# erikszasz/GaussianSplattingRegistration

Hardware: AMD Instinct MI355X
Metric: Gaussians/sec through HEM level + ICP iters/sec, 2x5M-splat pair (higher is better)
Workload: dtype f32 (HEM) / f64 (ICP)

## Files before the change

gaussiansplattingregistration_amd/csrc/hem_select.h:

```cpp
#pragma once
#include "hem_device.h"

namespace gsr {

struct ParentRec;
struct SelectArgs {
    const float4* A;
    const float4* geo;
    const float* Rs;
    const unsigned* plist;
    const unsigned* porder;
    int xcd;
    const int* nheavy;
    int own_lo, own_hi;
    const int* cellStart;
    const float4* Ac;
    const int* cellStartC;
    const int* cellStartI;
    const double* logtab;
    const int* irank;
    const unsigned* ipos;
    int n_irr;
    int ell;
    const GridParams* gp;
    int P;
    float colorThr2;
    float kldThr, tau2;
    const ParentRec* prec;
    unsigned* pcnt;
    unsigned* pcap;
    const int64_t* poff;
    unsigned* pair_child;
    float* pair_wl;
    const uint2* hitem;
    const int* hfirst;
    unsigned* part_cnt;
    int* hq;
    int heavy_blocks;
    const unsigned* part_p;
    unsigned long long cap_pairs;
    int* abort_p;
    int np;
    int2* rowlist;
};

enum { SEL_COUNT = 0, SEL_FILL = 1, SEL_SPARSE = 2 };
#define SEL_PART 8192
#define SEL_HEAVY_BLOCKS 2048
#define SEL_QCAP 256
#define SEL_U 3
#define SEL_MCAP 1024
#define SEL_ROWS 16
#define SEL_PAD (64 * SEL_U)

struct EllClip {
    float on;
    float k11, k12, k22, kr, im00, m01, m02, T;
};
struct ParentRec {
    f3 pm, pcol;
    s6 pinv;
    float det_p, inv_det_p, pweight, R, R2;
    float white;
    float u00, u01, u02, u11, u12, u22;
    float T1;
    EllClip ec;
    int js;
    int active;
    int selfq;
    float ey, ez;
    int rows;
};
static_assert(sizeof(ParentRec) == 160, "ParentRec is fetched as 40 dwords");

__device__ __forceinline__ float fast_sqrt(float x) { return __builtin_amdgcn_sqrtf(x); }

__device__ __forceinline__ int mbcnt64(unsigned long long mask, int base) {
    return (int)__builtin_amdgcn_mbcnt_hi((unsigned)(mask >> 32), __builtin_amdgcn_mbcnt_lo((unsigned)mask, (unsigned)base));
}
__device__ __forceinline__ unsigned long long uniform64(unsigned long long v) {
    return ((unsigned long long)(unsigned)__builtin_amdgcn_readfirstlane((int)(v >> 32)) << 32) |
           (unsigned)__builtin_amdgcn_readfirstlane((int)v);
}
__device__ __forceinline__ int wave_incl_scan(int v) {
    v += __builtin_amdgcn_update_dpp(0, v, 0x111, 0xf, 0xf, false);
    v += __builtin_amdgcn_update_dpp(0, v, 0x112, 0xf, 0xf, false);
    v += __builtin_amdgcn_update_dpp(0, v, 0x114, 0xf, 0xf, false);
    v += __builtin_amdgcn_update_dpp(0, v, 0x118, 0xf, 0xf, false);
    v += __builtin_amdgcn_update_dpp(0, v, 0x142, 0xa, 0xf, false);
    v += __builtin_amdgcn_update_dpp(0, v, 0x143, 0xc, 0xf, false);
    return v;
}

#ifdef GSR_SELECT_PROFILE
extern __device__ unsigned long long g_sel_prof[1024 * 16];
#define SEL_PROF_T(var) const unsigned long long var = __builtin_amdgcn_s_memtime()
#define SEL_PROF_ADD(slot, t0, lane) do { if ((lane) == 0) atomicAdd(&g_sel_prof[(blockIdx.x & 1023u) * 16 + (slot)], __builtin_amdgcn_s_memtime() - (t0)); } while (0)
#define SEL_PROF_CNT(slot, v, lane) do { if ((lane) == 0) atomicAdd(&g_sel_prof[(blockIdx.x & 1023u) * 16 + (slot)], (unsigned long long)(v)); } while (0)
#else
#define SEL_PROF_T(var)
#define SEL_PROF_ADD(slot, t0, lane)
#define SEL_PROF_CNT(slot, v, lane)
#endif

__device__ __forceinline__ bool kl_gate_rejects(float s2, float det_c, float det_p, float inv_det_p, float thr, const double* logtab,
                                                float* lf_out = nullptr, bool* exact_out = nullptr) {
    const float qf = det_c * inv_det_p;
    const float lf = __builtin_amdgcn_logf(qf) * 0.6931471805599453f;
    const float kf = 0.5f * (s2 - lf);
    const float margin = 1e-6f * (1.0f + fabsf(lf) + fabsf(s2));
    bool reject = kf > thr;
    const bool need_exact = !(qf >= 4.0f * FLT_MIN && qf <= 0.25f * FLT_MAX) || !(fabsf(s2) <= FLT_MAX) || !(fabsf(kf - thr) > margin);
    if (need_exact) {
        const float k = 0.5f * (s2 - glibc_logf_tab(det_c / det_p, logtab));
        reject = k > thr;
    }
    if (lf_out) *lf_out = lf;
    if (exact_out) *exact_out = need_exact;
    return reject;
}


template <bool IRR>
__device__ __forceinline__ void select_row_span(const SelectArgs& a, const GridParams& g, const f3& pm, const EllClip& ec, bool clip,
                                                float Ra2, int x0, int x1, int ry, int rz, int& s, int& len) {
    const bool edge = ry == 0 || ry == g.gy - 1 || rz == 0 || rz == g.gz - 1;
    const float ylo = ry == 0 ? -FLT_MAX : g.oy + ry * g.c - g.slack, yhi = ry == g.gy - 1 ? FLT_MAX : g.oy + (ry + 1) * g.c + g.slack;
    const float zlo = rz == 0 ? -FLT_MAX : g.oz + rz * g.c - g.slack, zhi = rz == g.gz - 1 ? FLT_MAX : g.oz + (rz + 1) * g.c + g.slack;
    const float dy = fmaxf(0.0f, fmaxf(ylo - pm.y, pm.y - yhi));
    const float dz = fmaxf(0.0f, fmaxf(zlo - pm.z, pm.z - zhi));
    const float rem = Ra2 - dy * dy - dz * dz;
    if (rem >= 0.0f) {
        const float hx = fast_sqrt(rem) * 1.00001f + g.slack;
        float lo = -hx, hi = hx;
        if (clip && !edge) {
            const float cy = 0.5f * (ylo + yhi) - pm.y, cz = 0.5f * (zlo + zhi) - pm.z;
            const float hy = 0.5f * (yhi - ylo), hz = 0.5f * (zhi - zlo);
            const float sc = fast_sqrt(fmaxf(0.0f, ec.k11 * cy * cy + 2.0f * ec.k12 * cy * cz + ec.k22 * cz * cz));
            const float smin = fmaxf(0.0f, sc * 0.999f - ec.kr * fast_sqrt(hy * hy + hz * hz));
            const float rem2 = ec.T - smin * smin;
            if (rem2 < 0.0f) {
                lo = 1.0f; hi = -1.0f;
            } else {
                const float w = fast_sqrt(rem2 * ec.im00) * 1.001f;
                const float t1 = ec.m01 * cy, t2 = ec.m02 * cz;
                const float xc = -(t1 + t2) * ec.im00;
                const float dl = (fabsf(ec.m01) * hy + fabsf(ec.m02) * hz) * ec.im00 * 1.001f;
                const float pad = g.slack + 1e-5f * fabsf(xc) + 1e-6f * (fabsf(t1) + fabsf(t2)) * ec.im00;
                lo = fmaxf(lo, xc - dl - w - pad);
                hi = fminf(hi, xc + dl + w + pad);
            }
        }
        if (lo <= hi) {
            int xa = cell_of(pm.x + lo, g.ox, g.inv_c, g.gx), xb = cell_of(pm.x + hi, g.ox, g.inv_c, g.gx);
            xa = xa < x0 ? x0 : xa;
            xb = xb > x1 ? x1 : xb;
            const int rowbase = (rz * g.gy + ry) * g.gx;
            int e;
            if (IRR) { s = a.cellStartI[rowbase + xa]; e = a.cellStartI[rowbase + xb + 1]; }
            else { s = a.cellStartC[rowbase + xa]; e = a.cellStartC[rowbase + xb + 1]; }
            len = e - s;
        }
    }
}

__device__ __forceinline__ void make_filter(const s6& Mf, float det_p, float kldThr, int ell, bool parent_regular, ParentRec& pr) {
    EllClip ec;
    ec.on = 0.0f; ec.k11 = ec.k12 = ec.k22 = ec.kr = ec.im00 = ec.m01 = ec.m02 = 0.0f; ec.T = __builtin_inff();
    pr.white = 0.0f;
    pr.u00 = pr.u01 = pr.u02 = pr.u11 = pr.u12 = pr.u22 = 0.0f;
    pr.T1 = __builtin_inff();
    pr.ey = pr.ez = __builtin_inff();
    const double thr2 = 2.0 * (double)kldThr;
    if (parent_regular && thr2 >= 0.0 && thr2 < 1e30) {
        const double m00 = Mf.e00, m01 = Mf.e01, m02 = Mf.e02, m11 = Mf.e11, m12 = Mf.e12, m22 = Mf.e22;
        double detM;
        const bool finite = fabs(m00) < 1e30 && fabs(m01) < 1e30 && fabs(m02) < 1e30 && fabs(m11) < 1e30 && fabs(m12) < 1e30 && fabs(m22) < 1e30;
        if (finite && spd_det64(m00, m01, m02, m11, m12, m22, detM)) {
            const double trM = m00 + m11 + m22;
            const double e2 = (m00 * m11 - m01 * m01) + (m00 * m22 - m02 * m02) + (m11 * m22 - m12 * m12);
            const double K = trM * e2 / detM * 1.000001;
            const double u = 5.9604644775390625e-8;
            const double theta = 6.1 * u * K + 2.0 * u;
            const double G = -(log(detM) + log((double)det_p)) + 2e-6;
            if (theta <= 0.25 && fabs(G) <= 1.0) {
                const double smin = (thr2 * (1.0 + 2.0 * u) + G + (double)GSR_DET_TOL + 3.2 * theta / (1.0 - theta) + 4e-5) / (1.0 - theta);
                const double T1 = smin * (1.0 + theta) * (1.0 + theta) * (1.0 + 1e-5);
                if (T1 > 0.0 && T1 < 1e30) {
                    const double u00 = sqrt(m00), u01 = m01 / u00, u02 = m02 / u00;
                    const double t11 = m11 - u01 * u01, u11 = sqrt(t11), u12 = (m12 - u01 * u02) / u11;
                    const double t22 = m22 - u02 * u02 - u12 * u12, u22 = sqrt(t22);
                    if (t11 > 0.0 && t22 > 0.0) {
                        pr.u00 = (float)u00; pr.u01 = (float)u01; pr.u02 = (float)u02; pr.u11 = (float)u11; pr.u12 = (float)u12; pr.u22 = (float)u22;
                        pr.T1 = (float)(T1 * (1.0 + 2.0 * u));
                        pr.white = 1.0f;
                        if (ell) {
                            const double Tc = T1 * (1.0 + theta) * (1.0 + theta) * (1.0 + 1e-4);
                            const double fk = 1.0 - 4.0 * theta - 2e-3;
                            const double im00 = 1.0 / m00;
                            const double k11 = (m11 - m01 * m01 * im00) * fk, k12 = (m12 - m01 * m02 * im00) * fk, k22 = (m22 - m02 * m02 * im00) * fk;
                            ec.k11 = (float)k11; ec.k12 = (float)k12; ec.k22 = (float)k22;
                            ec.kr = (float)(sqrt((k11 + k22) / fk) * 1.001);
                            ec.im00 = (float)(im00 * (1.0 + 4.0 * u));
                            ec.m01 = (float)m01; ec.m02 = (float)m02;
                            ec.T = (float)(Tc * (1.0 + 2.0 * u));
                            const bool ok = fk > 0.5 && k11 > 0.0 && k22 > 0.0 && k11 * k22 > k12 * k12 && ec.kr < FLT_MAX && ec.im00 < FLT_MAX && ec.T < FLT_MAX;
                            ec.on = ok ? 1.0f : 0.0f;
                            pr.ey = (float)(sqrt(fmax(0.0, Tc * (m00 * m22 - m02 * m02) / detM)) * 1.001);
                            pr.ez = (float)(sqrt(fmax(0.0, Tc * (m00 * m11 - m01 * m01) / detM)) * 1.001);
                        }
                    }
                }
            }
        }
    }
    pr.ec = ec;
}

__device__ __forceinline__ float white_smd(const float (&vc)[11], float cx, float cy, float cz) {
    const float dx = cx - vc[0], dy = cy - vc[1], dz = cz - vc[2];
    const float y2 = vc[8] * dz;
    const float y1 = __builtin_fmaf(vc[6], dy, vc[7] * dz);
    const float y0 = __builtin_fmaf(vc[3], dx, __builtin_fmaf(vc[4], dy, vc[5] * dz));
    return __builtin_fmaf(y0, y0, __builtin_fmaf(y1, y1, y2 * y2));
}

#define SEL_NP 4
#define SEL_TAG_SHIFT 30
#define SEL_TAG_MASK 0x3fffffffu

void launch_parent_prep(hipStream_t st, int P, const unsigned* plist, const float4* geo, const float* Rs, float kldThr, int ell, ParentRec* prec);
void launch_spans(hipStream_t st, const SelectArgs& sa);
int32_t launch_select(int mode, const SelectArgs& sa, hipStream_t st, hipStream_t aux, hipEvent_t ev_fork, hipEvent_t ev_join);
constexpr int SEL_WPB = 2;
void select_set_attributes();
int32_t select_profile(unsigned long long* out16, int32_t reset);

}
```

gaussiansplattingregistration_amd/csrc/hem_select.hip:

```cpp
#include "hem_select.h"

namespace gsr {

#ifdef GSR_SELECT_PROFILE
__device__ unsigned long long g_sel_prof[1024 * 16];
#endif
struct __attribute__((aligned(16))) ParLds {
    float4 r0;
    float4 r1;
    float4 r2;
    float4 r3;
    float R2;
    int js;
    int64_t base;
};
static_assert(sizeof(ParLds) == 80, "ParLds is read as four float4 and two 8-byte words");

#define SEL_Q3CAP 128
struct Q3 {
    unsigned *j, *rel;
    float *d2, *cd, *op, *det;
    int h, n;
};

__device__ __forceinline__ void select_stage3(const SelectArgs& a, const ParLds* par, int lane, int cnt, Q3& q3) {
    if (lane < cnt) {
        const int k = (q3.h + lane) & (SEL_Q3CAP - 1);
        const unsigned e = q3.j[k];
        const ParLds* pl = par + (e >> SEL_TAG_SHIFT);
        const float distanceDiff = sqrtf(q3.d2[k]);
        const float cdiff = sqrtf(q3.cd[k]);
        const float distWeight = expf(-distanceDiff * distanceDiff / a.tau2);
        const float colorInfluence = expf(-cdiff * cdiff / a.tau2);
        const float L = distWeight * q3.op[k] * colorInfluence * sqrtf(q3.det[k]);
        const int64_t dst = pl->base + (int64_t)q3.rel[k];
        a.pair_child[dst] = e & SEL_TAG_MASK;
        a.pair_wl[dst] = pl->r3.z * ref_clamp(L, FLT_MIN, 1e8f);
    }
    q3.h = (q3.h + cnt) & (SEL_Q3CAP - 1);
    q3.n -= cnt;
}

template <int MODE>
__device__ __forceinline__ void select_stage2(const SelectArgs& a, const ParLds* par, int lane, int cnt, const unsigned* q, int qh,
                                              unsigned& count_v, Q3& q3) {
    SEL_PROF_T(tp2);
    SEL_PROF_CNT(8, 1, lane); SEL_PROF_CNT(9, cnt, lane);
    bool acc = false;
    unsigned e = 0u;
    int k = 0;
    float d2 = 0.0f, cdiff = 0.0f, op = 0.0f, det_c = 0.0f;
    if (lane < cnt) {
        e = q[(qh + lane) & (SEL_QCAP - 1)];
        const int j = (int)(e & SEL_TAG_MASK);
        k = (int)(e >> SEL_TAG_SHIFT);
        const ParLds* pl = par + k;
        const float4 p0 = pl->r0, p1 = pl->r1;
        const float R2 = pl->R2;
        const float4* row = a.geo + 4 * (int64_t)j;
        float4 ca = row[0], cb = row[1], cc = row[2], cd = row[3];
        asm volatile("" : "+v"(ca.x), "+v"(ca.y), "+v"(ca.z), "+v"(ca.w), "+v"(cb.x), "+v"(cb.y), "+v"(cb.z), "+v"(cb.w),
                          "+v"(cc.x), "+v"(cc.y), "+v"(cc.z), "+v"(cc.w), "+v"(cd.x), "+v"(cd.y), "+v"(cd.z), "+v"(cd.w));
        const f3 cm = {ca.x, ca.y, ca.z};
        const f3 ccol = {cc.z, cc.w, cd.x};
        const f3 pm = {p0.x, p0.y, p0.z}, pcol = {p0.w, p1.x, p1.y};
        const f3 d = sub3(cm, pm);
        d2 = dot3(d, d);
        const f3 dc = sub3(ccol, pcol);
        cdiff = dot3(dc, dc);
        if (d2 < R2 && !(cdiff > a.colorThr2)) {
            const float4 p2 = pl->r2, p3 = pl->r3;
            const s6 ccov = {cb.x, cb.y, cb.z, cb.w, cc.x, cc.y};
            const s6 pinv = {p1.z, p1.w, p2.x, p2.y, p2.z, p2.w};
            det_c = cd.w;
            op = cd.y;
            const float smd = dot3(d, mul6(pinv, d));
            const float tr = trace_prod6(pinv, ccov);
            const float s2 = smd + tr - 3.0f;
            if (!kl_gate_rejects(s2, det_c, p3.x, p3.y, a.kldThr, a.logtab)) {
                const bool child_is_parent = (__float_as_uint(ca.w) & 1u) != 0u;
                acc = !(child_is_parent && j != pl->js);
            }
        }
    }
    const unsigned long long m = __ballot(acc);
    const int na = __popcll(m);
    SEL_PROF_CNT(15, na, lane);
    if (na == 0) { SEL_PROF_ADD(2, tp2, lane); return; }
    const int k_lo = __builtin_amdgcn_readfirstlane(k);
    const int k_hi = __builtin_amdgcn_readlane(k, __builtin_amdgcn_readfirstlane(cnt - 1));
    unsigned rel = 0u;
#pragma unroll
    for (int kk = 0; kk < SEL_NP; ++kk) {
        if (kk < k_lo || kk > k_hi) continue;
        const unsigned long long mk = __ballot(acc && k == kk);
        const unsigned ck = (unsigned)__builtin_amdgcn_readlane((int)count_v, kk);
        if (acc && k == kk) rel = ck + (unsigned)mbcnt64(mk, 0);
        if (lane == kk) count_v += (unsigned)__popcll(mk);
    }
    if (MODE == SEL_COUNT) { SEL_PROF_ADD(2, tp2, lane); return; }
    if (acc) {
        const int t = mbcnt64(m, q3.h + q3.n) & (SEL_Q3CAP - 1);
        q3.j[t] = e; q3.rel[t] = rel; q3.d2[t] = d2; q3.cd[t] = cdiff; q3.op[t] = op; q3.det[t] = det_c;
    }
    q3.n += na;
    __builtin_amdgcn_wave_barrier();
    if (q3.n >= 64) select_stage3(a, par, lane, 64, q3);
    __builtin_amdgcn_wave_barrier();
    SEL_PROF_ADD(2, tp2, lane);
}

__global__ __launch_bounds__(256) void k_parent_prep(int P, const unsigned* __restrict__ plist, const float4* __restrict__ geo,
                                                     const float* __restrict__ Rs, float kldThr, int ell, ParentRec* __restrict__ prec) {
    __shared__ ParentRec s_pr[4][64];
    const int lane = threadIdx.x & 63, wv = threadIdx.x >> 6;
    for (int base = blockIdx.x * blockDim.x + (threadIdx.x & ~63); base < P; base += gridDim.x * blockDim.x) {
        const int p = base + lane;
        if (p < P) {
        ParentRec pr;
        pr.js = (int)plist[p];
        const float4* prow = geo + 4 * (int64_t)pr.js;
        const float4 pa = prow[0], pb = prow[1], pc = prow[2], pd = prow[3];
        pr.pm = {pa.x, pa.y, pa.z};
        pr.det_p = pd.w;
        pr.inv_det_p = 1.0f / pd.w;
        const s6 pcov = {pb.x, pb.y, pb.z, pb.w, pc.x, pc.y};
        pr.pcol = {pc.z, pc.w, pd.x};
        pr.pweight = pd.z;
        pr.pinv = inverse6(pcov, pr.det_p);
        pr.R = Rs[pr.js];
        pr.R2 = pr.R * pr.R;
        make_filter(pr.pinv, pr.det_p, kldThr, ell, (__float_as_uint(pa.w) & 2u) != 0u, pr);
        const bool pm_finite = fabsf(pr.pm.x) <= FLT_MAX && fabsf(pr.pm.y) <= FLT_MAX && fabsf(pr.pm.z) <= FLT_MAX;
        pr.active = (pr.R2 > 0.0f && pm_finite) ? 1 : 0;
        pr.selfq = (pr.active && (__float_as_uint(pa.w) & 2u)) ? 1 : 0;
        pr.rows = 0;
        s_pr[wv][lane] = pr;
        }
        __builtin_amdgcn_wave_barrier();
        const int nrec = P - base < 64 ? P - base : 64;
        const float4* src = reinterpret_cast<const float4*>(s_pr[wv]);
        float4* dst = reinterpret_cast<float4*>(prec + base);
        for (int t = lane; t < nrec * (int)(sizeof(ParentRec) / 16); t += 64) dst[t] = src[t];
        __builtin_amdgcn_wave_barrier();
    }
}

template <int MODE, bool IRR>
__device__ __forceinline__ void select_scan(const SelectArgs& a, const GridParams& g, const ParentRec& pr, const ParLds* par, unsigned ktag,
                                            const float (&vc)[11], int lane, unsigned long long* bits, unsigned* q, int& qh, int& qn, unsigned& count_v,
                                            Q3& q3, unsigned& cum, unsigned lo, unsigned hi, const int2* rl, int lcnt) {
    const f3 pm = pr.pm;
    const EllClip& ec = pr.ec;
    const bool listed = rl != nullptr;
    bool clip = false;
    int x0 = 0, x1 = 0, y0 = 0, z0 = 0, ny = 1, nrows = lcnt;
    float Ra2 = 0.0f;
    if (!listed) {
        int vz;
        asm volatile("v_mov_b32 %0, 0" : "=v"(vz));
        const auto uni = [vz](int v) { return __builtin_amdgcn_readfirstlane(v + vz); };
        const auto unif = [vz](float v) { return __builtin_bit_cast(float, __builtin_amdgcn_readfirstlane(__builtin_bit_cast(int, v) + vz)); };
        const float Ra = unif(fabsf(pr.R) * 1.00001f + g.slack);
        clip = !IRR && ec.on != 0.0f;
        const float Ry = clip ? fminf(Ra, pr.ey + g.slack) : Ra, Rz = clip ? fminf(Ra, pr.ez + g.slack) : Ra;
        x0 = uni(cell_of(pm.x - Ra, g.ox, g.inv_c, g.gx)); x1 = uni(cell_of(pm.x + Ra, g.ox, g.inv_c, g.gx));
        y0 = uni(cell_of(pm.y - Ry, g.oy, g.inv_c, g.gy));
        const int y1 = uni(cell_of(pm.y + Ry, g.oy, g.inv_c, g.gy));
        z0 = uni(cell_of(pm.z - Rz, g.oz, g.inv_c, g.gz));
        const int z1 = uni(cell_of(pm.z + Rz, g.oz, g.inv_c, g.gz));
        ny = y1 - y0 + 1;
        nrows = ny * (z1 - z0 + 1);
        Ra2 = unif(Ra * Ra);
    }
    const bool white = !IRR && pr.white != 0.0f;
    SEL_PROF_CNT(10, nrows, lane);
    for (int rb = 0; rb < nrows; rb += 64) {
        SEL_PROF_T(tpr);
        SEL_PROF_CNT(11, 1, lane);
        const int r = rb + lane;
        int s = 0, len = 0;
        if (r < nrows) {
            if (listed) { const int2 e = rl[r]; s = e.x; len = e.y; }
            else select_row_span<IRR>(a, g, pm, ec, clip, Ra2, x0, x1, y0 + r % ny, z0 + r / ny, s, len);
        }
        len = len > 0 ? len : 0;
        const unsigned long long nz_m = __ballot(len > 0);
        if (nz_m == 0ull) continue;
        const int incl = wave_incl_scan(len);
        const int pre = incl - len;
        const int total = __builtin_amdgcn_readlane(incl, 63);
        const unsigned cum0 = cum;
        cum += (unsigned)total;
        if (hi <= cum0 || lo >= cum) continue;
        const int b_lo = lo > cum0 ? (int)(lo - cum0) : 0;
        const int b_hi = hi - cum0 < (unsigned)total ? (int)(hi - cum0) : total;
        const int nrb = __popcll(nz_m);
        const int below = mbcnt64(nz_m, 0);
        const int dst = len > 0 ? below : nrb + (lane - below);
        const int delta = __builtin_amdgcn_ds_permute(dst << 2, s - pre);
        SEL_PROF_ADD(1, tpr, lane);
        SEL_PROF_CNT(12, nrb, lane); SEL_PROF_CNT(13, total, lane);
        for (int seg0 = b_lo; seg0 < b_hi; seg0 += SEL_MCAP) {
            const int rel = pre - seg0;
            const bool mine = len > 0 && rel >= 0 && rel < SEL_MCAP;
            if (mine) atomicOr(&bits[rel >> 6], 1ull << (rel & 63));
            int rows_before = __popcll(__ballot(len > 0 && rel < 0));
            __builtin_amdgcn_wave_barrier();
            const int seg_end = b_hi < seg0 + SEL_MCAP ? b_hi : seg0 + SEL_MCAP;
            for (int t0 = seg0; t0 < seg_end; t0 += 64 * SEL_U) {
                SEL_PROF_CNT(14, 1, lane);
                SEL_PROF_T(tps);
                float4 ca[SEL_U];
                int jj[SEL_U];
                int left[SEL_U];
#pragma unroll
                for (int u = 0; u < SEL_U; ++u) {
                    const int c0 = t0 + 64 * u;
                    const unsigned long long word = uniform64(bits[(c0 - seg0) >> 6]);
                    const int row = mbcnt64(word >> 1, rows_before - 1 + (int)(word & 1ull));
                    rows_before += __popcll(word);
                    left[u] = seg_end - c0;
                    const int k = c0 + lane + __builtin_amdgcn_ds_bpermute(row << 2, delta);
                    if (IRR) { jj[u] = lane < left[u] ? (int)a.ipos[k] : pr.js; ca[u] = a.A[jj[u]]; }
                    else { jj[u] = k; ca[u] = a.Ac[k]; }
                }
#pragma unroll
                for (int u = 0; u < SEL_U; ++u) {
                    if (left[u] <= 0) continue;
                    const f3 cm = {ca[u].x, ca[u].y, ca[u].z};
                    bool in;
                    if (white) {
                        in = !(white_smd(vc, cm.x, cm.y, cm.z) > vc[9]);
                    } else {
                        const f3 dq = sub3(pm, cm);
                        in = dot3(dq, dq) < pr.R2;
                    }
                    if (!IRR) {
                        in = in && (__float_as_uint(ca[u].w) & 2u);
                        jj[u] = (int)(__float_as_uint(ca[u].w) >> 2);
                    } else {
                        in = in && (!(__float_as_uint(ca[u].w) & 1u) || jj[u] == pr.js);
                    }
                    in = in && lane < left[u];
                    const unsigned long long m = __ballot(in);
                    if (m == 0ull) continue;
                    if (in) q[mbcnt64(m, qh + qn) & (SEL_QCAP - 1)] = (unsigned)jj[u] | ktag;
                    qn += __popcll(m);
                }
                __builtin_amdgcn_wave_barrier();
                SEL_PROF_ADD(4, tps, lane);
                while (qn >= 64) {
                    select_stage2<MODE>(a, par, lane, 64, q, qh, count_v, q3);
                    qh = (qh + 64) & (SEL_QCAP - 1);
                    qn -= 64;
                }
                __builtin_amdgcn_wave_barrier();
            }
            if (mine) bits[rel >> 6] = 0ull;
            __builtin_amdgcn_wave_barrier();
        }
    }
}

__device__ __forceinline__ void select_fill_par(const SelectArgs& a, int p, int64_t base, ParLds* slot) {
    const float4* r = reinterpret_cast<const float4*>(a.prec + p);
    const float4 r0 = r[0], r1 = r[1], r2 = r[2], r3 = r[3];
    slot->r0 = r0; slot->r1 = r1; slot->r2 = r2; slot->r3 = r3;
    slot->R2 = a.prec[p].R2; slot->js = a.prec[p].js; slot->base = base;
}

template <int MODE>
__device__ __forceinline__ void select_parent(const SelectArgs& a, const GridParams& g, int p, int k, unsigned lo, unsigned hi, int lane,
                                              const ParLds* par, unsigned* q, int& qh, int& qn, unsigned long long* bits, unsigned& count_v, Q3& q3) {
    SEL_PROF_T(tp0);
    ParentRec pr;
    {
        typedef unsigned u16v __attribute__((ext_vector_type(16)));
        typedef unsigned u8v __attribute__((ext_vector_type(8)));
        u16v w0, w1; u8v w2;
        const ParentRec* rp = a.prec + p;
        asm volatile("s_load_dwordx16 %0, %3, 0x0\n\ts_load_dwordx16 %1, %3, 0x40\n\ts_load_dwordx8 %2, %3, 0x80\n\ts_waitcnt lgkmcnt(0)"
                     : "=&s"(w0), "=&s"(w1), "=&s"(w2) : "s"(rp) : "memory");
        unsigned raw[40];
        static_assert(sizeof(raw) == sizeof(ParentRec), "the three scalar loads cover the record");
#pragma unroll
        for (int i = 0; i < 16; ++i) { raw[i] = w0[i]; raw[16 + i] = w1[i]; }
#pragma unroll
        for (int i = 0; i < 8; ++i) raw[32 + i] = w2[i];
        __builtin_memcpy(&pr, raw, sizeof(pr));
    }
    float vc[11];
    {
        const float src[11] = {pr.pm.x, pr.pm.y, pr.pm.z, pr.u00, pr.u01, pr.u02, pr.u11, pr.u12, pr.u22, pr.T1, 0.0f};
#pragma unroll
        for (int i = 0; i < 11; ++i) asm volatile("v_mov_b32 %0, %1" : "=v"(vc[i]) : "s"(src[i]));
    }
    const unsigned ktag = (unsigned)k << SEL_TAG_SHIFT;
    unsigned cum = 0;
    if (pr.selfq) {
        cum = 1u;
        if (lo == 0u) {
            if (lane == 0) q[(qh + qn) & (SEL_QCAP - 1)] = (unsigned)pr.js | ktag;
            qn += 1;
        }
        __builtin_amdgcn_wave_barrier();
        if (qn >= 64) {
            select_stage2<MODE>(a, par, lane, 64, q, qh, count_v, q3);
            qh = (qh + 64) & (SEL_QCAP - 1);
            qn -= 64;
        }
    }
    if (pr.active) {
        const int cA = pr.rows & 0xff, cB = (pr.rows >> 8) & 0xff;
        const int2* rlp = (a.rowlist != nullptr && pr.rows < 0) ? a.rowlist + (int64_t)p * (2 * SEL_ROWS) : nullptr;
        select_scan<MODE, false>(a, g, pr, par, ktag, vc, lane, bits, q, qh, qn, count_v, q3, cum, lo, hi,
                                 rlp != nullptr && cA <= SEL_ROWS ? rlp : nullptr, cA);
        if (a.n_irr > 0) select_scan<MODE, true>(a, g, pr, par, ktag, vc, lane, bits, q, qh, qn, count_v, q3, cum, lo, hi,
                                                 rlp != nullptr && cB <= SEL_ROWS ? rlp + SEL_ROWS : nullptr, cB);
    }
    SEL_PROF_ADD(0, tp0, lane);
    SEL_PROF_CNT(7, 1, lane);
}

template <int MODE>
__device__ __forceinline__ void select_flush(const SelectArgs& a, const ParLds* par, int lane, const unsigned* q, int& qh, int& qn,
                                             unsigned& count_v, Q3& q3) {
    while (qn > 0) {
        const int c = qn < 64 ? qn : 64;
        select_stage2<MODE>(a, par, lane, c, q, qh, count_v, q3);
        qh = (qh + c) & (SEL_QCAP - 1);
        qn -= c;
    }
    SEL_PROF_T(tp3);
    if ((MODE == SEL_FILL || MODE == SEL_SPARSE) && q3.n > 0) select_stage3(a, par, lane, q3.n, q3);
    SEL_PROF_ADD(3, tp3, lane);
    __builtin_amdgcn_wave_barrier();
}

template <int MODE, int WPB, bool QUEUE>
__global__ __launch_bounds__(64 * WPB) void k_select(SelectArgs a) {
    __shared__ unsigned s_q[WPB][SEL_QCAP];
    __shared__ unsigned s_q3u[WPB][2][SEL_Q3CAP];
    __shared__ float s_q3f[WPB][4][SEL_Q3CAP];
    __shared__ unsigned long long s_bits[WPB][SEL_MCAP / 64 + SEL_U];
    __shared__ ParLds s_par[WPB][SEL_NP];
    const int lane = threadIdx.x & 63, wv = __builtin_amdgcn_readfirstlane((int)(threadIdx.x >> 6));
    a.logtab = k_logf_tab;
    if (lane < SEL_MCAP / 64 + SEL_U) s_bits[wv][lane] = 0ull;
    unsigned* q = s_q[wv];
    ParLds* par = s_par[wv];
    Q3 q3 = {s_q3u[wv][0], s_q3u[wv][1], s_q3f[wv][0], s_q3f[wv][1], s_q3f[wv][2], s_q3f[wv][3], 0, 0};
    __builtin_amdgcn_wave_barrier();
    const GridParams g = *a.gp;
    int qh = 0, qn = 0;

    if constexpr (QUEUE) {
        const int n_items = a.hq[0];
        const unsigned part = *a.part_p;
        int item = (int)blockIdx.x * WPB + wv;
        while (item < n_items) {
            const uint2 it = a.hitem[item];
            const int p = __builtin_amdgcn_readfirstlane((int)a.porder[it.x]);
            const unsigned lo = (unsigned)__builtin_amdgcn_readfirstlane((int)(it.y * part));
            const unsigned hi = lo + part > lo ? lo + part : 0xffffffffu;
            int64_t base = 0;
            if (MODE == SEL_SPARSE) base = a.poff[p] + lo;
            if (MODE == SEL_SPARSE && a.cap_pairs && (unsigned long long)base + part > a.cap_pairs) {
                if (lane == 0) { a.part_cnt[item] = 0u; *a.abort_p = 1; }
                int nxt0 = 0;
                if (lane == 0) nxt0 = atomicAdd(&a.hq[1], 1);
                item = __builtin_amdgcn_readfirstlane(nxt0);
                continue;
            }
            if (MODE == SEL_FILL) {
                base = a.poff[p];
                for (int k = a.hfirst[p]; k < item; ++k) base += a.part_cnt[k];
            }
            unsigned count_v = 0u;
            if (lane == 0) select_fill_par(a, p, base, par);
            __builtin_amdgcn_wave_barrier();
            select_parent<MODE>(a, g, p, 0, lo, hi, lane, par, q, qh, qn, s_bits[wv], count_v, q3);
            select_flush<MODE>(a, par, lane, q, qh, qn, count_v, q3);
            if (lane == 0 && (MODE == SEL_COUNT || MODE == SEL_SPARSE)) {
                a.part_cnt[item] = count_v;
                atomicAdd(&a.pcnt[p], count_v);
            }
            int nxt = 0;
            if (lane == 0) nxt = atomicAdd(&a.hq[1], 1);
            item = __builtin_amdgcn_readfirstlane(nxt);
            __builtin_amdgcn_wave_barrier();
        }
    } else {
        SEL_PROF_T(tpk);
        const int np = a.np;
        const int ppb = WPB * np;
        const int nheavy = a.nheavy ? *a.nheavy : 0;
        const int nblk = (a.P + ppb - 1) / ppb;
        const int hb = ((nheavy + ppb - 1) / ppb + 7) & ~7;
        const int bid = block_slot((int)blockIdx.x, nblk, hb < nblk ? hb : nblk, a.xcd);
        if (bid < 0) return;
        const int slot0 = (bid * WPB + wv) * np;
        int p_v = -1;
        if (lane < np) {
            const int slot = slot0 + lane;
            if (slot < a.P && !(a.heavy_blocks > 0 && slot < nheavy)) {
                const int p = a.porder ? (int)a.porder[slot] : slot;
                if (p < a.own_lo || p >= a.own_hi) {
                    if (MODE == SEL_COUNT || MODE == SEL_SPARSE) a.pcnt[p] = 0u;
                } else {
                    const int64_t base = (MODE == SEL_FILL || MODE == SEL_SPARSE) ? a.poff[p] : 0;
                    if (MODE == SEL_SPARSE && a.cap_pairs && (unsigned long long)base + a.pcap[p] > a.cap_pairs) {
                        a.pcnt[p] = 0u; *a.abort_p = 1;
                    } else {
                        p_v = p;
                        select_fill_par(a, p, base, par + lane);
                    }
                }
            }
        }
        unsigned long long todo = __ballot(p_v >= 0);
        unsigned count_v = 0u;
        __builtin_amdgcn_wave_barrier();
        SEL_PROF_ADD(5, tpk, lane);
        while (todo != 0ull) {
            const int k = __builtin_ctzll(todo);
            todo &= todo - 1ull;
            const int p = __builtin_amdgcn_readlane(p_v, k);
            select_parent<MODE>(a, g, p, k, 0u, 0xffffffffu, lane, par, q, qh, qn, s_bits[wv], count_v, q3);
        }
        SEL_PROF_T(tpf);
        select_flush<MODE>(a, par, lane, q, qh, qn, count_v, q3);
        SEL_PROF_ADD(6, tpf, lane);
        if (p_v >= 0 && (MODE == SEL_COUNT || MODE == SEL_SPARSE)) a.pcnt[p_v] = count_v;
    }
}

__global__ __launch_bounds__(256) void k_spans(SelectArgs a) {
    const int sub = threadIdx.x & 15;
    const int p = (int)(((int64_t)blockIdx.x * blockDim.x + threadIdx.x) >> 4);
    if (p >= a.P) return;
    unsigned long long scanned = 0;
    int selfq = 0;
    int nA = 0, nB = 0;
    if (p >= a.own_lo && p < a.own_hi) {
        const GridParams g = *a.gp;
        const float4* rq = reinterpret_cast<const float4*>(a.prec + p);
        float4 q0 = rq[0], q3 = rq[3], q6 = rq[6], q7 = rq[7], q8 = rq[8], q9 = rq[9];
        asm volatile("" : "+v"(q0.x), "+v"(q0.y), "+v"(q0.z), "+v"(q3.w), "+v"(q6.y), "+v"(q6.z), "+v"(q6.w), "+v"(q7.x), "+v"(q7.y), "+v"(q7.z), "+v"(q7.w),
                          "+v"(q8.x), "+v"(q8.y), "+v"(q8.w), "+v"(q9.x), "+v"(q9.y), "+v"(q9.z));
        static_assert(offsetof(ParentRec, R) == 60 && offsetof(ParentRec, ec) == 100 && offsetof(ParentRec, active) == 140 && offsetof(ParentRec, ey) == 148,
                      "k_spans reads the record by offsets");
        const f3 pm = {q0.x, q0.y, q0.z};
        const EllClip ec = {q6.y, q6.z, q6.w, q7.x, q7.y, q7.z, q7.w, q8.x, q8.y};
        struct { float R, ey, ez; int active; } rv = {q3.w, q9.y, q9.z, __float_as_int(q8.w)};
        const auto* rp = &rv;
        selfq = __float_as_int(q9.x);
        const unsigned gsh = (unsigned)(threadIdx.x & 48);
        const auto keep_span = [&](int pass, int s, int len, int& n) {
            const unsigned gm = (unsigned)(__ballot(len > 0) >> gsh) & 0xffffu;
            if (len > 0 && a.rowlist) {
                const int pos = n + __popc(gm & ((1u << sub) - 1u));
                if (pos < SEL_ROWS) a.rowlist[((int64_t)p * 2 + pass) * SEL_ROWS + pos] = make_int2(s, len);
            }
            n += __popc(gm);
        };
        if (rp->active) {
            const float Ra = fabsf(rp->R) * 1.00001f + g.slack;
            const float Ra2 = Ra * Ra;
            const int x0 = cell_of(pm.x - Ra, g.ox, g.inv_c, g.gx), x1 = cell_of(pm.x + Ra, g.ox, g.inv_c, g.gx);
            {
                const bool clip = ec.on != 0.0f;
                const float Ry = clip ? fminf(Ra, rp->ey + g.slack) : Ra, Rz = clip ? fminf(Ra, rp->ez + g.slack) : Ra;
                const int y0 = cell_of(pm.y - Ry, g.oy, g.inv_c, g.gy), y1 = cell_of(pm.y + Ry, g.oy, g.inv_c, g.gy);
                const int z0 = cell_of(pm.z - Rz, g.oz, g.inv_c, g.gz), z1 = cell_of(pm.z + Rz, g.oz, g.inv_c, g.gz);
                const int ny = y1 - y0 + 1, nrows = ny * (z1 - z0 + 1);
                for (int r = sub; r < nrows; r += 16) {
                    int s = 0, len = 0;
                    select_row_span<false>(a, g, pm, ec, clip, Ra2, x0, x1, y0 + r % ny, z0 + r / ny, s, len);
                    scanned += (unsigned long long)(len > 0 ? len : 0);
                    keep_span(0, s, len, nA);
                }
            }
            if (a.n_irr > 0) {
                const int y0 = cell_of(pm.y - Ra, g.oy, g.inv_c, g.gy), y1 = cell_of(pm.y + Ra, g.oy, g.inv_c, g.gy);
                const int z0 = cell_of(pm.z - Ra, g.oz, g.inv_c, g.gz), z1 = cell_of(pm.z + Ra, g.oz, g.inv_c, g.gz);
                const int ny = y1 - y0 + 1, nrows = ny * (z1 - z0 + 1);
                for (int r = sub; r < nrows; r += 16) {
                    int s = 0, len = 0;
                    select_row_span<true>(a, g, pm, ec, false, Ra2, x0, x1, y0 + r % ny, z0 + r / ny, s, len);
                    scanned += (unsigned long long)(len > 0 ? len : 0);
                    keep_span(1, s, len, nB);
                }
            }
        }
    }
    for (int o = 8; o > 0; o >>= 1) scanned += __shfl_xor(scanned, o);
    if (selfq) scanned += 1ull;
    if (sub == 0) {
        a.pcap[p] = (unsigned)(scanned > 0xffffffffull ? 0xffffffffull : scanned);
        if (a.rowlist) const_cast<ParentRec*>(a.prec)[p].rows = (int)(0x80000000u | (unsigned)(nA > SEL_ROWS ? 0xff : nA) | ((unsigned)(nB > SEL_ROWS ? 0xff : nB) << 8));
    }
}

void launch_parent_prep(hipStream_t st, int P, const unsigned* plist, const float4* geo, const float* Rs, float kldThr, int ell, ParentRec* prec) {
    hipLaunchKernelGGL(k_parent_prep, dim3(stride_grid(P)), dim3(256), 0, st, P, plist, geo, Rs, kldThr, ell, prec);
}
void launch_spans(hipStream_t st, const SelectArgs& sa) {
    hipLaunchKernelGGL(k_spans, dim3(ceil_div(sa.P, 16)), dim3(256), 0, st, sa);
}
template <int MODE>
static int32_t launch_select_mode(const SelectArgs& sa, hipStream_t st, hipStream_t aux, hipEvent_t ev_fork, hipEvent_t ev_join) {
    constexpr int WPB = SEL_WPB;
    if (sa.heavy_blocks) {
        GSR_HIP(hipEventRecord(ev_fork, st)); GSR_HIP(hipStreamWaitEvent(aux, ev_fork, 0));
        hipLaunchKernelGGL((k_select<MODE, WPB, true>), dim3(sa.heavy_blocks), dim3(64 * WPB), 0, aux, sa);
        GSR_HIP(hipEventRecord(ev_join, aux));
    }
    hipLaunchKernelGGL((k_select<MODE, WPB, false>), dim3(8 * ceil_div(ceil_div(sa.P, WPB * sa.np), 8)), dim3(64 * WPB), 0, st, sa);
    if (sa.heavy_blocks) GSR_HIP(hipStreamWaitEvent(st, ev_join, 0));
    return GSR_OK;
}
int32_t launch_select(int mode, const SelectArgs& sa, hipStream_t st, hipStream_t aux, hipEvent_t ev_fork, hipEvent_t ev_join) {
    if (mode == SEL_SPARSE) return launch_select_mode<SEL_SPARSE>(sa, st, aux, ev_fork, ev_join);
    if (mode == SEL_COUNT) return launch_select_mode<SEL_COUNT>(sa, st, aux, ev_fork, ev_join);
    return launch_select_mode<SEL_FILL>(sa, st, aux, ev_fork, ev_join);
}
void select_set_attributes() {}
int32_t select_profile(unsigned long long* out16, int32_t reset) {
#ifdef GSR_SELECT_PROFILE
    static unsigned long long h[1024 * 16];
    if (out16) {
        if (hipMemcpyFromSymbol(h, HIP_SYMBOL(g_sel_prof), sizeof(h)) != hipSuccess) return GSR_E_HIP;
        for (int k = 0; k < 16; ++k) { out16[k] = 0; for (int b = 0; b < 1024; ++b) out16[k] += h[b * 16 + k]; }
    }
    if (reset) { memset(h, 0, sizeof(h)); if (hipMemcpyToSymbol(HIP_SYMBOL(g_sel_prof), h, sizeof(h)) != hipSuccess) return GSR_E_HIP; }
    return GSR_OK;
#else
    (void)out16; (void)reset;
    return GSR_E_INVALID;
#endif
}

}
```

Before: 576.2 million.

## Rematerialize select kernel constants from kernarg/scalar loads to cut SGPR pressure

Stops holding the full ParentRec, GridParams and many SelectArgs pointers live across the select kernel. It reloads them on demand through inline s_load from the kernarg segment and the parent record at fixed offsets. Per-wave LDS is regrouped into one struct, and the COUNT mode no longer allocates the stage-3 queues. The aim is lower scalar register pressure, fewer spills and possibly smaller LDS use for higher occupancy, at the cost of repeated scalar loads with waits and brittle offset-dependent asm.

```diff
diff --git a/gaussiansplattingregistration_amd/csrc/hem_select.h b/gaussiansplattingregistration_amd/csrc/hem_select.h
--- a/gaussiansplattingregistration_amd/csrc/hem_select.h
+++ b/gaussiansplattingregistration_amd/csrc/hem_select.h
@@ -121,8 +121,7 @@
 }
 
 
-template <bool IRR>
-__device__ __forceinline__ void select_row_span(const SelectArgs& a, const GridParams& g, const f3& pm, const EllClip& ec, bool clip,
+__device__ __forceinline__ void select_row_span(const int* __restrict__ tab, const GridParams& g, const f3& pm, const EllClip& ec, bool clip,
                                                 float Ra2, int x0, int x1, int ry, int rz, int& s, int& len) {
     const bool edge = ry == 0 || ry == g.gy - 1 || rz == 0 || rz == g.gz - 1;
     const float ylo = ry == 0 ? -FLT_MAX : g.oy + ry * g.c - g.slack, yhi = ry == g.gy - 1 ? FLT_MAX : g.oy + (ry + 1) * g.c + g.slack;
@@ -156,10 +155,8 @@
             xa = xa < x0 ? x0 : xa;
             xb = xb > x1 ? x1 : xb;
             const int rowbase = (rz * g.gy + ry) * g.gx;
-            int e;
-            if (IRR) { s = a.cellStartI[rowbase + xa]; e = a.cellStartI[rowbase + xb + 1]; }
-            else { s = a.cellStartC[rowbase + xa]; e = a.cellStartC[rowbase + xb + 1]; }
-            len = e - s;
+            s = tab[rowbase + xa];
+            len = tab[rowbase + xb + 1] - s;
         }
     }
 }
diff --git a/gaussiansplattingregistration_amd/csrc/hem_select.hip b/gaussiansplattingregistration_amd/csrc/hem_select.hip
--- a/gaussiansplattingregistration_amd/csrc/hem_select.hip
+++ b/gaussiansplattingregistration_amd/csrc/hem_select.hip
@@ -1,4 +1,6 @@
 #include "hem_select.h"
+
+#include <type_traits>
 
 namespace gsr {
 
@@ -21,6 +23,15 @@
     unsigned *j, *rel;
     float *d2, *cd, *op, *det;
     int h, n;
+};
+
+struct __attribute__((aligned(8))) WaveLdsCount {
+    unsigned long long bits[SEL_MCAP / 64 + SEL_U];
+    unsigned q[SEL_QCAP];
+};
+struct __attribute__((aligned(8))) WaveLds : WaveLdsCount {
+    unsigned j[SEL_Q3CAP], rel[SEL_Q3CAP];
+    float d2[SEL_Q3CAP], cd[SEL_Q3CAP], op[SEL_Q3CAP], det[SEL_Q3CAP];
 };
 
 __device__ __forceinline__ void select_stage3(const SelectArgs& a, const ParLds* par, int lane, int cnt, Q3& q3) {
@@ -146,22 +157,61 @@
     }
 }
 
+struct ParentS {
+    float R2, white;
+    int js, active, selfq;
+    float ey, ez;
+    int rows;
+};
+typedef unsigned sel_u2v __attribute__((ext_vector_type(2)));
+typedef unsigned sel_u4v __attribute__((ext_vector_type(4)));
+typedef unsigned sel_u8v __attribute__((ext_vector_type(8)));
+static_assert(offsetof(ParentRec, R) == 60 && offsetof(ParentRec, R2) == 64 && offsetof(ParentRec, T1) == 96 && offsetof(ParentRec, ec) == 100 &&
+              offsetof(ParentRec, js) == 136 && offsetof(ParentRec, selfq) == 144 && offsetof(ParentRec, rows) == 156 && sizeof(EllClip) == 36 &&
+              offsetof(GridParams, gz) == 32, "select_parent / select_row_consts read the records by offsets");
+
+#define SEL_KARG(m1, v1, m2, v2)                                                                                                     \
+    asm volatile("s_load_dwordx2 %0, %2, %3\n\ts_load_dwordx2 %1, %2, %4\n\ts_waitcnt lgkmcnt(0)" : "=&s"(v1), "=&s"(v2)          \
+                 : "s"(__builtin_amdgcn_kernarg_segment_ptr()), "n"(offsetof(SelectArgs, m1)), "n"(offsetof(SelectArgs, m2)) : "memory")
+
+#define SEL_KARG1(m1, v1)                                                                                                            \
+    asm volatile("s_load_dwordx2 %0, %1, %2\n\ts_waitcnt lgkmcnt(0)" : "=s"(v1) : "s"(__builtin_amdgcn_kernarg_segment_ptr()), "n"(offsetof(SelectArgs, m1)) : "memory")
+
+template <bool IRR>
+__device__ __forceinline__ void select_row_consts(int p, GridParams& g, EllClip& ec, float& R, const int*& tab) {
+    sel_u8v g0, e0; sel_u2v g1; unsigned e1, r;
+    const GridParams* gp; const ParentRec* rp;
+    SEL_KARG(gp, gp, prec, rp);
+    if (IRR) SEL_KARG1(cellStartI, tab); else SEL_KARG1(cellStartC, tab);
+    rp += p;
+    asm volatile("s_load_dwordx8 %0, %5, 0x0\n\ts_load_dwordx2 %1, %5, 0x20\n\ts_load_dwordx8 %2, %6, 0x64\n\ts_load_dword %3, %6, 0x84\n\t"
+                 "s_load_dword %4, %6, 0x3c\n\ts_waitcnt lgkmcnt(0)"
+                 : "=&s"(g0), "=&s"(g1), "=&s"(e0), "=&s"(e1), "=&s"(r) : "s"(gp), "s"(rp) : "memory");
+    const auto f = [](unsigned v) { return __builtin_bit_cast(float, v); };
+    g.ox = f(g0[0]); g.oy = f(g0[1]); g.oz = f(g0[2]); g.c = f(g0[3]); g.inv_c = f(g0[4]); g.slack = f(g0[5]);
+    g.gx = (int)g0[6]; g.gy = (int)g0[7]; g.gz = (int)g1[0]; g.ncells = (int)g1[1];
+    ec.on = f(e0[0]); ec.k11 = f(e0[1]); ec.k12 = f(e0[2]); ec.k22 = f(e0[3]); ec.kr = f(e0[4]); ec.im00 = f(e0[5]); ec.m01 = f(e0[6]); ec.m02 = f(e0[7]);
+    ec.T = f(e1);
+    R = f(r);
+}
+
 template <int MODE, bool IRR>
-__device__ __forceinline__ void select_scan(const SelectArgs& a, const GridParams& g, const ParentRec& pr, const ParLds* par, unsigned ktag,
+__device__ __forceinline__ void select_scan(const SelectArgs& a, int p, const ParentS& pr, const ParLds* par, unsigned ktag,
                                             const float (&vc)[11], int lane, unsigned long long* bits, unsigned* q, int& qh, int& qn, unsigned& count_v,
                                             Q3& q3, unsigned& cum, unsigned lo, unsigned hi, const int2* rl, int lcnt) {
-    const f3 pm = pr.pm;
-    const EllClip& ec = pr.ec;
+    const f3 pm = {vc[0], vc[1], vc[2]};
     const bool listed = rl != nullptr;
     bool clip = false;
     int x0 = 0, x1 = 0, y0 = 0, z0 = 0, ny = 1, nrows = lcnt;
     float Ra2 = 0.0f;
     if (!listed) {
+        GridParams g; EllClip ec; float R; const int* tab;
+        select_row_consts<IRR>(p, g, ec, R, tab);
         int vz;
         asm volatile("v_mov_b32 %0, 0" : "=v"(vz));
         const auto uni = [vz](int v) { return __builtin_amdgcn_readfirstlane(v + vz); };
         const auto unif = [vz](float v) { return __builtin_bit_cast(float, __builtin_amdgcn_readfirstlane(__builtin_bit_cast(int, v) + vz)); };
-        const float Ra = unif(fabsf(pr.R) * 1.00001f + g.slack);
+        const float Ra = unif(fabsf(R) * 1.00001f + g.slack);
         clip = !IRR && ec.on != 0.0f;
         const float Ry = clip ? fminf(Ra, pr.ey + g.slack) : Ra, Rz = clip ? fminf(Ra, pr.ez + g.slack) : Ra;
         x0 = uni(cell_of(pm.x - Ra, g.ox, g.inv_c, g.gx)); x1 = uni(cell_of(pm.x + Ra, g.ox, g.inv_c, g.gx));
@@ -182,7 +232,11 @@
         int s = 0, len = 0;
         if (r < nrows) {
             if (listed) { const int2 e = rl[r]; s = e.x; len = e.y; }
-            else select_row_span<IRR>(a, g, pm, ec, clip, Ra2, x0, x1, y0 + r % ny, z0 + r / ny, s, len);
+        }
+        if (!listed) {
+            GridParams g; EllClip ec; float R; const int* tab;
+            select_row_consts<IRR>(p, g, ec, R, tab);
+            if (r < nrows) select_row_span(tab, g, pm, ec, clip, Ra2, x0, x1, y0 + r % ny, z0 + r / ny, s, len);
         }
         len = len > 0 ? len : 0;
         const unsigned long long nz_m = __ballot(len > 0);
@@ -271,28 +325,25 @@
 }
 
 template <int MODE>
-__device__ __forceinline__ void select_parent(const SelectArgs& a, const GridParams& g, int p, int k, unsigned lo, unsigned hi, int lane,
+__device__ __forceinline__ void select_parent(const SelectArgs& a, int p, int k, unsigned lo, unsigned hi, int lane,
                                               const ParLds* par, unsigned* q, int& qh, int& qn, unsigned long long* bits, unsigned& count_v, Q3& q3) {
     SEL_PROF_T(tp0);
-    ParentRec pr;
-    {
-        typedef unsigned u16v __attribute__((ext_vector_type(16)));
-        typedef unsigned u8v __attribute__((ext_vector_type(8)));
-        u16v w0, w1; u8v w2;
-        const ParentRec* rp = a.prec + p;
-        asm volatile("s_load_dwordx16 %0, %3, 0x0\n\ts_load_dwordx16 %1, %3, 0x40\n\ts_load_dwordx8 %2, %3, 0x80\n\ts_waitcnt lgkmcnt(0)"
-                     : "=&s"(w0), "=&s"(w1), "=&s"(w2) : "s"(rp) : "memory");
-        unsigned raw[40];
-        static_assert(sizeof(raw) == sizeof(ParentRec), "the three scalar loads cover the record");
-#pragma unroll
-        for (int i = 0; i < 16; ++i) { raw[i] = w0[i]; raw[16 + i] = w1[i]; }
-#pragma unroll
-        for (int i = 0; i < 8; ++i) raw[32 + i] = w2[i];
-        __builtin_memcpy(&pr, raw, sizeof(pr));
-    }
+    ParentS pr;
+    const int2* rowlist;
     float vc[11];
     {
-        const float src[11] = {pr.pm.x, pr.pm.y, pr.pm.z, pr.u00, pr.u01, pr.u02, pr.u11, pr.u12, pr.u22, pr.T1, 0.0f};
+        sel_u4v w0, w3; sel_u8v w1; sel_u2v w2; unsigned t1;
+        const ParentRec* rp;
+        SEL_KARG(prec, rp, rowlist, rowlist);
+        rp += p;
+        asm volatile("s_load_dwordx4 %0, %5, 0x0\n\ts_load_dwordx8 %1, %5, 0x40\n\ts_load_dword %2, %5, 0x60\n\ts_load_dwordx2 %3, %5, 0x88\n\t"
+                     "s_load_dwordx4 %4, %5, 0x90\n\ts_waitcnt lgkmcnt(0)"
+                     : "=&s"(w0), "=&s"(w1), "=&s"(t1), "=&s"(w2), "=&s"(w3) : "s"(rp) : "memory");
+        const auto f = [](unsigned v) { return __builtin_bit_cast(float, v); };
+        pr.R2 = f(w1[0]); pr.white = f(w1[1]);
+        pr.js = (int)w2[0]; pr.active = (int)w2[1];
+        pr.selfq = (int)w3[0]; pr.ey = f(w3[1]); pr.ez = f(w3[2]); pr.rows = (int)w3[3];
+        const unsigned src[11] = {w0[0], w0[1], w0[2], w1[2], w1[3], w1[4], w1[5], w1[6], w1[7], t1, 0u};
 #pragma unroll
         for (int i = 0; i < 11; ++i) asm volatile("v_mov_b32 %0, %1" : "=v"(vc[i]) : "s"(src[i]));
     }
@@ -313,10 +364,12 @@
     }
     if (pr.active) {
         const int cA = pr.rows & 0xff, cB = (pr.rows >> 8) & 0xff;
-        const int2* rlp = (a.rowlist != nullptr && pr.rows < 0) ? a.rowlist + (int64_t)p * (2 * SEL_ROWS) : nullptr;
-        select_scan<MODE, false>(a, g, pr, par, ktag, vc, lane, bits, q, qh, qn, count_v, q3, cum, lo, hi,
+        const int2* rlp = (rowlist != nullptr && pr.rows < 0) ? rowlist + (int64_t)p * (2 * SEL_ROWS) : nullptr;
+        select_scan<MODE, false>(a, p, pr, par, ktag, vc, lane, bits, q, qh, qn, count_v, q3, cum, lo, hi,
                                  rlp != nullptr && cA <= SEL_ROWS ? rlp : nullptr, cA);
-        if (a.n_irr > 0) select_scan<MODE, true>(a, g, pr, par, ktag, vc, lane, bits, q, qh, qn, count_v, q3, cum, lo, hi,
+        int n_irr;
+        asm volatile("s_load_dword %0, %1, %2\n\ts_waitcnt lgkmcnt(0)" : "=s"(n_irr) : "s"(__builtin_amdgcn_kernarg_segment_ptr()), "n"(offsetof(SelectArgs, n_irr)) : "memory");
+        if (n_irr > 0) select_scan<MODE, true>(a, p, pr, par, ktag, vc, lane, bits, q, qh, qn, count_v, q3, cum, lo, hi,
                                                  rlp != nullptr && cB <= SEL_ROWS ? rlp + SEL_ROWS : nullptr, cB);
     }
     SEL_PROF_ADD(0, tp0, lane);
@@ -340,54 +393,69 @@
 
 template <int MODE, int WPB, bool QUEUE>
 __global__ __launch_bounds__(64 * WPB) void k_select(SelectArgs a) {
-    __shared__ unsigned s_q[WPB][SEL_QCAP];
-    __shared__ unsigned s_q3u[WPB][2][SEL_Q3CAP];
-    __shared__ float s_q3f[WPB][4][SEL_Q3CAP];
-    __shared__ unsigned long long s_bits[WPB][SEL_MCAP / 64 + SEL_U];
+    typedef typename std::conditional<MODE == SEL_COUNT, WaveLdsCount, WaveLds>::type Wave;
+    __shared__ Wave s_w[WPB];
     __shared__ ParLds s_par[WPB][SEL_NP];
     const int lane = threadIdx.x & 63, wv = __builtin_amdgcn_readfirstlane((int)(threadIdx.x >> 6));
     a.logtab = k_logf_tab;
-    if (lane < SEL_MCAP / 64 + SEL_U) s_bits[wv][lane] = 0ull;
-    unsigned* q = s_q[wv];
+    Wave* w = s_w + wv;
+    if (lane < SEL_MCAP / 64 + SEL_U) w->bits[lane] = 0ull;
+    unsigned* q = w->q;
     ParLds* par = s_par[wv];
-    Q3 q3 = {s_q3u[wv][0], s_q3u[wv][1], s_q3f[wv][0], s_q3f[wv][1], s_q3f[wv][2], s_q3f[wv][3], 0, 0};
+    Q3 q3 = {};
+    if constexpr (MODE != SEL_COUNT) q3 = {w->j, w->rel, w->d2, w->cd, w->op, w->det, 0, 0};
     __builtin_amdgcn_wave_barrier();
-    const GridParams g = *a.gp;
     int qh = 0, qn = 0;
 
     if constexpr (QUEUE) {
-        const int n_items = a.hq[0];
-        const unsigned part = *a.part_p;
         int item = (int)blockIdx.x * WPB + wv;
-        while (item < n_items) {
-            const uint2 it = a.hitem[item];
-            const int p = __builtin_amdgcn_readfirstlane((int)a.porder[it.x]);
+        for (;;) {
+            int* hq; const unsigned* part_p;
+            SEL_KARG(hq, hq, part_p, part_p);
+            if (item >= __builtin_amdgcn_readfirstlane(hq[0])) break;
+            const uint2* hitem; const unsigned* porder;
+            SEL_KARG(hitem, hitem, porder, porder);
+            const uint2 it = hitem[item];
+            const unsigned part = (unsigned)__builtin_amdgcn_readfirstlane((int)*part_p);
+            const int p = __builtin_amdgcn_readfirstlane((int)porder[it.x]);
             const unsigned lo = (unsigned)__builtin_amdgcn_readfirstlane((int)(it.y * part));
             const unsigned hi = lo + part > lo ? lo + part : 0xffffffffu;
             int64_t base = 0;
-            if (MODE == SEL_SPARSE) base = a.poff[p] + lo;
-            if (MODE == SEL_SPARSE && a.cap_pairs && (unsigned long long)base + part > a.cap_pairs) {
-                if (lane == 0) { a.part_cnt[item] = 0u; *a.abort_p = 1; }
-                int nxt0 = 0;
-                if (lane == 0) nxt0 = atomicAdd(&a.hq[1], 1);
-                item = __builtin_amdgcn_readfirstlane(nxt0);
-                continue;
-            }
-            if (MODE == SEL_FILL) {
-                base = a.poff[p];
-                for (int k = a.hfirst[p]; k < item; ++k) base += a.part_cnt[k];
+            if (MODE == SEL_SPARSE || MODE == SEL_FILL) {
+                const int64_t* poff; unsigned* part_cnt;
+                SEL_KARG(poff, poff, part_cnt, part_cnt);
+                if (MODE == SEL_SPARSE) {
+                    base = (int64_t)uniform64((unsigned long long)poff[p]) + lo;
+                    unsigned long long cap_pairs;
+                    SEL_KARG1(cap_pairs, cap_pairs);
+                    if (cap_pairs && (unsigned long long)base + part > cap_pairs) {
+                        int nxt0 = 0;
+                        if (lane == 0) { part_cnt[item] = 0u; *a.abort_p = 1; nxt0 = atomicAdd(&hq[1], 1); }
+                        item = __builtin_amdgcn_readfirstlane(nxt0);
+                        continue;
+                    }
+                } else {
+                    base = poff[p];
+                    for (int k = a.hfirst[p]; k < item; ++k) base += part_cnt[k];
+                }
             }
             unsigned count_v = 0u;
             if (lane == 0) select_fill_par(a, p, base, par);
             __builtin_amdgcn_wave_barrier();
-            select_parent<MODE>(a, g, p, 0, lo, hi, lane, par, q, qh, qn, s_bits[wv], count_v, q3);
+            select_parent<MODE>(a, p, 0, lo, hi, lane, par, q, qh, qn, w->bits, count_v, q3);
             select_flush<MODE>(a, par, lane, q, qh, qn, count_v, q3);
-            if (lane == 0 && (MODE == SEL_COUNT || MODE == SEL_SPARSE)) {
-                a.part_cnt[item] = count_v;
-                atomicAdd(&a.pcnt[p], count_v);
-            }
             int nxt = 0;
-            if (lane == 0) nxt = atomicAdd(&a.hq[1], 1);
+            if (lane == 0) {
+                if (MODE == SEL_COUNT || MODE == SEL_SPARSE) {
+                    unsigned* part_cnt; unsigned* pcnt;
+                    SEL_KARG(part_cnt, part_cnt, pcnt, pcnt);
+                    SEL_KARG(hitem, hitem, porder, porder);
+                    part_cnt[item] = count_v;
+                    atomicAdd(&pcnt[porder[hitem[item].x]], count_v);
+                }
+                SEL_KARG1(hq, hq);
+                nxt = atomicAdd(&hq[1], 1);
+            }
             item = __builtin_amdgcn_readfirstlane(nxt);
             __builtin_amdgcn_wave_barrier();
         }
@@ -427,12 +495,16 @@
             const int k = __builtin_ctzll(todo);
             todo &= todo - 1ull;
             const int p = __builtin_amdgcn_readlane(p_v, k);
-            select_parent<MODE>(a, g, p, k, 0u, 0xffffffffu, lane, par, q, qh, qn, s_bits[wv], count_v, q3);
+            select_parent<MODE>(a, p, k, 0u, 0xffffffffu, lane, par, q, qh, qn, w->bits, count_v, q3);
         }
         SEL_PROF_T(tpf);
         select_flush<MODE>(a, par, lane, q, qh, qn, count_v, q3);
         SEL_PROF_ADD(6, tpf, lane);
-        if (p_v >= 0 && (MODE == SEL_COUNT || MODE == SEL_SPARSE)) a.pcnt[p_v] = count_v;
+        if (MODE == SEL_COUNT || MODE == SEL_SPARSE) {
+            unsigned* pcnt;
+            SEL_KARG1(pcnt, pcnt);
+            if (p_v >= 0) pcnt[p_v] = count_v;
+        }
     }
 }
 
@@ -477,7 +549,7 @@
                 const int ny = y1 - y0 + 1, nrows = ny * (z1 - z0 + 1);
                 for (int r = sub; r < nrows; r += 16) {
                     int s = 0, len = 0;
-                    select_row_span<false>(a, g, pm, ec, clip, Ra2, x0, x1, y0 + r % ny, z0 + r / ny, s, len);
+                    select_row_span(a.cellStartC, g, pm, ec, clip, Ra2, x0, x1, y0 + r % ny, z0 + r / ny, s, len);
                     scanned += (unsigned long long)(len > 0 ? len : 0);
                     keep_span(0, s, len, nA);
                 }
@@ -488,7 +560,7 @@
                 const int ny = y1 - y0 + 1, nrows = ny * (z1 - z0 + 1);
                 for (int r = sub; r < nrows; r += 16) {
                     int s = 0, len = 0;
-                    select_row_span<true>(a, g, pm, ec, false, Ra2, x0, x1, y0 + r % ny, z0 + r / ny, s, len);
+                    select_row_span(a.cellStartI, g, pm, ec, false, Ra2, x0, x1, y0 + r % ny, z0 + r / ny, s, len);
                     scanned += (unsigned long long)(len > 0 ? len : 0);
                     keep_span(1, s, len, nB);
                 }
```

Result: no change. 579.2 million, median of 6 (+0.5%).
